# andgoldschmidt/MPC4quantum

Hardware: AMD Instinct MI355X
Metric: MPC horizon-steps/sec across batch (3-level transmon, T=40) (higher is better)
Workload: dtype f64

## Files before the change

### mpc4quantum_amd/csrc/build.py

```python
import argparse
import os
import re
import subprocess
import sys
from concurrent.futures import ThreadPoolExecutor

HERE = os.path.dirname(os.path.abspath(__file__))
PKG = os.path.dirname(HERE)
OBJ = os.path.join(HERE, "build")
LIB = os.path.join(PKG, "libm4q_hip.so")
LIB_GEN = os.path.join(PKG, "libm4q_hip_gen.so")
HIPCC = os.environ.get("HIPCC", "/opt/rocm/bin/hipcc")
COMMON = ["--offload-arch=gfx950", "-O3", "-std=c++17", "-fPIC", "-fvisibility=hidden", "-Wno-unused-command-line-argument"]
HEADERS = ["m4q_device.h", "m4q_dpp_gen.h", "m4q_mpc.h", "m4q_tile.h", "m4q_tile3.h", "m4q_tile_opnd.h", "m4q_rollout_pair.h", "m4q_args.h", "m4q_paths.h", "m4q_lift.h", "m4q_noise.h", "m4q_fit.h", "m4q_fit_qr.h", "m4q_online.h", "m4q_grad.h", "m4q_plant_lin.h", "m4q_plant_qp.h", "m4q_plant_step.h", "m4q_rollout_multi.h", "m4q_robust_host.h", "m4q_feedback.h", "m4q_observe.h", "m4q_shapes.inc",
           os.path.join("..", "..", "include", "m4q.h")]
STAMP = os.path.join(OBJ, "flags.stamp")


def shapes():
    txt = open(os.path.join(HERE, "m4q_shapes.inc")).read()
    return [(int(a), int(b), int(c), "plant-only" in rest)
            for a, b, c, rest in re.findall(r"^M4Q_SHAPE\((\d+),\s*(\d+),\s*(\d+)\)(.*)$", txt, re.M)]


def stale(target, sources):
    if not os.path.exists(target):
        return True
    t = os.path.getmtime(target)
    return any(os.path.getmtime(s) > t for s in sources)


def run(cmd):
    res = subprocess.run(cmd, stdout=subprocess.PIPE, stderr=subprocess.STDOUT, text=True)
    if res.returncode != 0:
        sys.stderr.write(" ".join(cmd) + "\n" + res.stdout)
        raise RuntimeError("hipcc failed")
    return res.stdout


def build(force=False, jobs=None, extra=()):
    os.makedirs(OBJ, exist_ok=True)
    hdrs = [os.path.join(HERE, h) for h in HEADERS]
    gen = os.path.join(HERE, "m4q_dpp_gen.h")
    if stale(gen, [os.path.join(HERE, "gen_dpp.py")]):
        text = run([sys.executable, os.path.join(HERE, "gen_dpp.py")])
        if not os.path.exists(gen) or open(gen).read() != text:
            with open(gen, "w") as f:
                f.write(text)
    want = " ".join(extra)
    have = open(STAMP).read() if os.path.exists(STAMP) else None
    if have != want:
        force = True
    jobs_list = []
    objs = []
    gen_objs = []
    for nx, nu, order, plant_only in shapes():
        obj = os.path.join(OBJ, "kernels_%d_%d_%d.o" % (nx, nu, order))
        objs.append(obj)
        src = os.path.join(HERE, "m4q_kernels.hip")
        dims = ["-DM4Q_NX=%d" % nx, "-DM4Q_NU=%d" % nu, "-DM4Q_ORDER=%d" % order]
        if force or stale(obj, [src] + hdrs):
            jobs_list.append([HIPCC] + COMMON + list(extra) + dims + (["-DM4Q_PLANT_ONLY"] if plant_only else []) + ["-c", src, "-o", obj])
        d = {4: 2, 9: 3, 16: 4}.get(nx)
        if d and not plant_only:
            gobj = os.path.join(OBJ, "kernelsg_%d_%d_%d.o" % (nx, nu, order))
            gen_objs.append(gobj)
            if force or stale(gobj, [src] + hdrs):
# ... 35 lines not shown
```

### mpc4quantum_amd/csrc/m4q_capi.hip

```cpp
#include <hip/hip_runtime.h>
#include <dlfcn.h>
#include <rccl/rccl.h>

#include <algorithm>
#include <cfloat>
#include <cmath>
#include <complex>
#include <cstdlib>
#include <cstdarg>
#include <cstdio>
#include <cstring>
#include <deque>
#include <mutex>
#include <string>
#include <vector>

#include "../../include/m4q.h"
#include "m4q_args.h"
#include "m4q_lift.h"
#include "m4q_robust_host.h"

namespace m4q {
struct cplx { double re, im; };
}
// ... 824 lines not shown
  s->noise_seed = seed;
  s->noise_member_base = member_base;
  s->noise_mode = mode;
  return 0;
}

int m4q_session_sync(m4q_session* s) {
  if (!s) return fail(M4Q_E_BADARG, "m4q_session_sync: null session");
  HIP_TRY(hipStreamSynchronize(s->stream));
  return check_watchdog(s);
}

int m4q_session_set_codes(m4q_session* s, const int32_t* codes) {
  if (!s || !codes) return fail(M4Q_E_BADARG, "m4q_session_set_codes: bad argument");
  HIP_TRY(hipMemcpyAsync(s->f[M4Q_F_CODES].p, codes, (size_t)s->B * 4, hipMemcpyHostToDevice, s->stream));
  HIP_TRY(hipStreamSynchronize(s->stream));
  return check_watchdog(s);
}

int m4q_session_kernel_ms(m4q_session* s, double* total_ms, int32_t* launches) {
  if (!s) return fail(M4Q_E_BADARG, "m4q_session_kernel_ms: null session");
  HIP_TRY(hipStreamSynchronize(s->stream));
  double tot = s->folded_ms;
  int n = s->folded_n;
  s->folded_ms = 0.0;
  s->folded_n = 0;
  for (auto& pr : s->pending) {
    float ms = 0.f;
    HIP_TRY(hipEventElapsedTime(&ms, pr.first, pr.second));
    tot += ms;
    ++n;
    (void)hipEventDestroy(pr.first);
    (void)hipEventDestroy(pr.second);
  }
  s->pending.clear();
  if (total_ms) *total_ms = tot;
  if (launches) *launches = n;
  return check_watchdog(s);
}

int m4q_session_qp_stats(m4q_session* s, int64_t* out6) {
  if (!s || !out6) return fail(M4Q_E_BADARG, "m4q_session_qp_stats: bad argument");
  HIP_TRY(hipStreamSynchronize(s->stream));
  unsigned long long q[24];
  HIP_TRY(hipMemcpy(q, s->queue.p, sizeof(q), hipMemcpyDeviceToHost));
  for (int i = 0; i < 6; ++i) out6[i] = (int64_t)q[1 + i];
  if (std::getenv("M4Q_QP_TRACE"))
    fprintf(stderr, "m4q: exact QP: %llu row sweeps in %llu wavefront passes (x4 rows = %llu): lane efficiency %.2f\n", q[2], q[7],
            4 * q[7], q[7] ? (double)q[2] / (4.0 * (double)q[7]) : 0.0);
  if (std::getenv("M4Q_PHASE_TRACE")) {
    static const char* names[16] = {"draw/resume", "backward | exact: adjoint pass", "forward", "handover", "line search", "step done (plant)", "publish",
                                    "passes", "guess update", "passes with a line search",
                                    "step: bookkeeping, us | exact: pinned sweep", "step: plant to xs | exact: policy rollout",
                                    "exact: ratio rollout", "step: exit, rest | exact: blend", "exact: open rollout",
                                    "exact: bookkeeping + copies"};
    unsigned long long tot = 0;
    for (int i = 0; i < 16; ++i) tot += (i == 7 || i == 9) ? 0 : q[8 + i];
    for (int i = 0; i < 16; ++i)
      fprintf(stderr, "m4q phase %-44s %14llu %s  %5.1f %%\n", names[i], q[8 + i], (i == 7 || i == 9) ? "     " : "ticks",
              (i != 7 && i != 9 && tot) ? 100.0 * (double)q[8 + i] / (double)tot : 0.0);
  }
  return check_watchdog(s);
}

int m4q_session_info(const m4q_session* s, int64_t* hbm_bytes, int32_t* grid, int32_t* lds_bytes) {
  if (!s) return fail(M4Q_E_BADARG, "m4q_session_info: null session");
  int64_t tot = 0;
  for (int i = 0; i < M4Q_F_COUNT; ++i) tot += (int64_t)s->f[i].bytes;
  tot += (int64_t)(s->wsXg.bytes + s->wsUg.bytes + s->wsG.bytes);
  if (hbm_bytes) *hbm_bytes = tot;
  const m4q::Path path = s->path();
  if (grid) *grid = path == m4q::PATH_SG ? s->grid_sg : s->grid;
  if (lds_bytes) *lds_bytes = s->mpc_ops->mpc_lds_bytes(s->prob.plant_kind, path, (s->prob.qp_flags & M4Q_QP_EXACT_BOX) != 0);
  return 0;
}

int m4q_linearize_batch(int32_t B, int32_t dim_x, int32_t dim_u, int32_t order, int32_t T, const double* models,
                        int32_t model_per_instance, const double* X, const double* U, double* A_ls, double* B_ls,
                        double* Delta_ls) {
  const m4q::ShapeOps* sh = find_shape(dim_x, dim_u, order);
  if (!sh) return fail(M4Q_E_UNSUPPORTED, "no kernel for dim_x=%d dim_u=%d order=%d", dim_x, dim_u, order);
  if (B <= 0 || T <= 0 || !models || !X || !U || !A_ls || !B_ls || !Delta_ls) return fail(M4Q_E_BADARG, "m4q_linearize_batch: bad argument");
  if (int rc = need_device()) return rc;
  const size_t n = dim_x, m = dim_u, P = sh->np, BT = (size_t)B * T;
  const Extent mdl(B, model_per_instance, n * n * (1 + P));
  Stage st;
  m4q::LinArgs a{};
  a.B = B; a.T = T;
  a.models = st.in<cplx>(models, mdl.count); a.model_stride = mdl.stride;
  a.X = st.in<cplx>(X, BT * n); a.U = st.in<double>(U, BT * m);
  a.A_ls = st.out<cplx>(A_ls, BT * n * n); a.B_ls = st.out<cplx>(B_ls, BT * n * m); a.D_ls = st.out<cplx>(Delta_ls, BT * n);
  if (st.error()) return st.error();
  return st.finish(sh->launch_linearize(a, nullptr), "linearize");
}

int m4q_quad_program_batch(int32_t B, int32_t dim_x, int32_t dim_u, int32_t T, int32_t qp_flags, double sat, double du,
                           const double* x_init, const double* X_bm, const double* U_bm, int32_t bm_per_instance,
                           const double* Q_ls, const double* R_ls, const double* A_ls, const double* B_ls,
                           const double* Delta_ls, const double* u_prev, double* X_opt, double* U_opt, double* cost,
                           double* gains) {
  const m4q::ShapeOps* sh = find_shape_any_order(dim_x, dim_u);
  if (!sh) return fail(M4Q_E_UNSUPPORTED, "no kernel for dim_x=%d dim_u=%d", dim_x, dim_u);
  if (B <= 0 || T <= 0 || !x_init || !X_bm || !U_bm || !Q_ls || !R_ls || !A_ls || !B_ls || !X_opt || !U_opt || !cost)
    return fail(M4Q_E_BADARG, "m4q_quad_program_batch: bad argument");
  if (!(sat > 0)) return fail(M4Q_E_BADARG, "sat must be positive");
  if (int rc = check_qp_flags(qp_flags)) return rc;
  if (int rc = need_device()) return rc;
  const size_t n = dim_x, m = dim_u, BT = (size_t)B * T, BT1 = (size_t)B * (T + 1);
  const Extent xbm(B, bm_per_instance, (size_t)(T + 1) * n), ubm(B, bm_per_instance, (size_t)T * m);
  Stage st;
  m4q::QpArgs a{};
  a.B = B; a.T = T; a.flags = qp_flags; a.sat = sat; a.du = du;
  a.x_init = st.in<cplx>(x_init, (size_t)B * n);
// ... 1188 lines not shown
```

### mpc4quantum_amd/csrc/m4q_kernels.hip

```cpp
#define M4Q_KERNEL_TU 1
#include "m4q_args.h"
#include "m4q_mpc.h"
#include "m4q_feedback.h"
#include "m4q_fit.h"
#include "m4q_fit_qr.h"
#include "m4q_online.h"
#include "m4q_grad.h"
#include "m4q_plant_lin.h"
#include "m4q_plant_qp.h"
#include "m4q_noise.h"
#include "m4q_observe.h"
#include "m4q_tile3.h"

#ifndef M4Q_NX
#error "compile with -DM4Q_NX -DM4Q_NU -DM4Q_ORDER"
#endif
#if defined(M4Q_PLANT_ONLY) || defined(M4Q_VARIANT_GEN)
#define M4Q_NO_AUX 1
#endif

#define M4Q_CAT_(a, b, c, d) a##b##_##c##_##d
#define M4Q_CAT(a, b, c, d) M4Q_CAT_(a, b, c, d)

namespace m4q {
namespace M4Q_CAT(shape_, M4Q_NX, M4Q_NU, M4Q_ORDER) {

constexpr int NX = M4Q_NX;
constexpr int NU = M4Q_NU;
constexpr int ORDER = M4Q_ORDER;
constexpr int DD = (NX == 4) ? 2 : (NX == 9) ? 3 : (NX == 16) ? 4 : 1;
constexpr bool SQUARE = DD * DD == NX;
constexpr int DQ = fourth_root(NX);
constexpr bool QUARTIC = DQ > 0;
constexpr int NP = PowTab<NU, ORDER>::NP;
constexpr int PITCH = ModelPitch<NX>::value;
constexpr int MODEL_ELEMS = (1 + NP) * NX * PITCH;
constexpr int SCRATCH_ELEMS = (SQUARE ? DD * DD : 0) + 2 * NX;
constexpr int ROWS = 4;
constexpr bool HAS_TILE = SQUARE && ORDER == 1 && NX - 1 <= 8;
constexpr bool HAS_SG = SQUARE && ORDER == 1 && NX == 16;

constexpr int WAVES = NX <= 9 ? 2 : 1;
#define M4Q_OCC __attribute__((amdgpu_waves_per_eu(WAVES, 8)))

extern __shared__ __align__(16) unsigned char m4q_lds_raw[];

template <int N, class S>
__device__ __forceinline__ void stage_model(S* dst, const M4Q_GLOBAL S* src, int jj) {
  constexpr int W = N * (1 + NP);
#pragma unroll 1
  for (int e = jj; e < N * W; e += 16) {
    const int i = e / W;
    const int pk = e - i * W;
    const int p = pk / N;
    const int k = pk - p * N;
    dst[ModelPitch<N>::at(p, i, k)] = gld(src, e);
  }
}

struct LaneGeo {
  int g, jj, j;
  bool lane_ok;
  __device__ __forceinline__ LaneGeo() {
    const int lane = threadIdx.x;
    g = lane >> 4;
// ... 76 lines not shown

template <int NS>
struct ExactTile {
  static constexpr bool enabled = true;
  const double* lds_models;
  volatile M4Q_LDS double* tgb; volatile M4Q_LDS int* tiw; volatile M4Q_LDS double* tpin;
  GView Xg, Ug, gains;
  const double* Q; const double* Qf; const double* R;
  unsigned sX, sU, sG;
  int g, jj;
  __device__ __forceinline__ void sweep(int T, const Window& win, const PinCtx<NU>& pin, bool going) const {
    if (jj == 0) {
      tiw[g * TILE_IO_WORDS + 0] = going ? 1 : 0;
      tiw[g * TILE_IO_WORDS + 1] = (int)win.xbm.off;
      tiw[g * TILE_IO_WORDS + 2] = (int)win.ubm.off;
      tiw[g * TILE_IO_WORDS + 3] = (int)pin.stat.off;
#pragma unroll
      for (int k = 0; k < NU; ++k) { tpin[g * TILE_PIN_DOUBLES + k] = pin.lo0[k]; tpin[g * TILE_PIN_DOUBLES + 3 + k] = pin.hi0[k]; }
    }
    wave_sync();
    TileBackwardB<NS, NU, ORDER, true> ts;
    const int mb = ts.L.mb;
    const int dm = mb - g;
    ts.mdl = lds_models + mb * model_elems<NS>();
    ts.T = T;
    ts.Xg = Xg; ts.Xg.off = Xg.off + (unsigned)(dm * (int)(sX * sizeof(double)));
    ts.Ug = Ug; ts.Ug.off = Ug.off + (unsigned)(dm * (int)(sU * sizeof(double)));
    ts.gains = gains; ts.gains.off = gains.off + (unsigned)(dm * (int)(sG * sizeof(double)));
    ts.xbm = win.xbm; ts.xbm.off = (unsigned)tiw[mb * TILE_IO_WORDS + 1];
    ts.ubm = win.ubm; ts.ubm.off = (unsigned)tiw[mb * TILE_IO_WORDS + 2];
    ts.stat = pin.stat; ts.stat.off = (unsigned)tiw[mb * TILE_IO_WORDS + 3];
    ts.sat = pin.box.sat;
    ts.Q = Q; ts.Qf = Qf; ts.R = R;
    ts.gb = tgb + mb * TILE_GB_DOUBLES;
    const bool run_t = tiw[mb * TILE_IO_WORDS + 0] != 0;
    ts.backward(run_t);
    wave_sync();
  }
};

constexpr int TC_MIN_N = 8;
constexpr int XCUTS[] = {4, 7, 12};
constexpr int NXC = (int)(sizeof(XCUTS) / sizeof(int));
constexpr int WAVES_SG = 2;
constexpr int WAVES_TILE = 2;
template <class S, int PLANT, bool EXACT, bool TL, bool TILE, bool SG>
constexpr PrioMap prio_map() {
  if (TILE && !EXACT && NX == 9 && PLANT == PLANT_HAMILTONIAN) return PrioMap{0, 1, 1, 1, 1, 1};
  return PrioMap{0, 0, 0, 0, 0, 0};
}
template <bool EXACT>
constexpr bool shift_in_update() {
  return !EXACT;
}
#if defined(M4Q_DEV_PHASE_CLOCK)
#define M4Q_PHASE_FLUSH() if (threadIdx.x == 0) { for (int i = 0; i < 16; ++i) __hip_atomic_fetch_add((M4Q_GLOBAL unsigned long long*)kargs()->queue + 8 + i, pc.acc[i], __ATOMIC_RELAXED, __HIP_MEMORY_SCOPE_AGENT); }
#else
#define M4Q_PHASE_FLUSH()
#endif
#define M4Q_PHASE_DECL PhaseClock pc;
#define M4Q_PHASE_MARK(i) pc.mark(i);
#define M4Q_PHASE_MARK_CLIP(i) if constexpr (!EXACT) pc.mark(i);
template <class S, int PLANT, bool EXACT, bool TL = false, bool TILE = false, bool SG = false>
__global__ __launch_bounds__(64) __attribute__((amdgpu_waves_per_eu(SG ? WAVES_SG : TILE ? WAVES_TILE : WAVES, 8))) void mpc_kernel(MpcArgs) {
  static_assert(!TL || (sizeof(S) == sizeof(double) && SQUARE), "the traceless path is a real path of a d x d density matrix");
  static_assert(!TILE || (TL && !EXACT && ORDER == 1), "tile sweep: clipped solve on the traceless real coordinates, order-1 libraries");
  static_assert(!SG || (TL && !TILE && !EXACT && ORDER == 1), "shared generators: the clipped traceless kernel of an order-1 library");
  constexpr int NS = TL ? NX - 1 : NX;
  using Prov = FusedProv<S, NS, NU, ORDER, SG>;
  cplx* scratch = reinterpret_cast<cplx*>(m4q_lds_raw);
  S* lds = reinterpret_cast<S*>(scratch + ROWS * SCRATCH_ELEMS);
  const LaneGeo L;
  const int g = L.g, jj = L.jj;
  const int j = jj < NS ? jj : NS - 1;
  const int jio = L.j;
  const bool lane_ok = jj < NS, lane_io = L.lane_ok;
  double tau = 0.0;
  constexpr bool QTR = cost_transposed<S, NS, EXACT>();
  constexpr int MODEL_K = SG ? NS * ModelPitch<NS>::value : model_elems<NS>(), COST_K = cost_elems<NS>() + (QTR ? 2 * NS * NS : 0);
  S* mdl = lds + g * MODEL_K;
  S* mdn = lds + ROWS * MODEL_K;
  scratch += g * SCRATCH_ELEMS;
  S* ldsQ = lds + model_lds_elems<NS, SG>();
  double* ldsW = reinterpret_cast<double*>(ldsQ + COST_K);
  volatile M4Q_LDS unsigned long long* wd_slot = (volatile M4Q_LDS unsigned long long*)(ldsW + WLS_DOUBLES);
  RowStash<S> stash;
  stash.w = (volatile M4Q_LDS int*)(ldsW + WLS_DOUBLES + 1);
  stash.xm = stash_x_in_scratch<S, SG>() ? (volatile M4Q_LDS double*)m4q_lds_raw : (volatile M4Q_LDS double*)(stash.w + ROWS * STASH_INTS);
  volatile M4Q_LDS double* tgb = stash.xm + 64 * 2;
  volatile M4Q_LDS int* tiw = (volatile M4Q_LDS int*)(tgb + ROWS * TILE_GB_DOUBLES);
  volatile M4Q_LDS double* tpin = (volatile M4Q_LDS double*)(tiw + ROWS * TILE_IO_WORDS);
  volatile M4Q_LDS double* timg = (volatile M4Q_LDS double*)(tiw + ROWS * TILE_IO_WORDS);
  int T0, flags;
  bool ls_diag, two_phase;
  int n_pieces;
  auto piece_cut = [](int i) __attribute__((always_inline)) {
    int v = 2;
#pragma unroll
    for (int k = 0; k < NXC; ++k)
      if (i == k + 2) v = XCUTS[k];
    return v;
  };
  auto piece_of = [&](int begin, int step_begin) __attribute__((always_inline)) {
    int ph = begin == step_begin ? 0 : 1;
#pragma unroll
    for (int k = 0; k < NXC; ++k)
      if (begin == XCUTS[k] && begin != step_begin) ph = k + 2;
    return ph;
  };
  {
    KArgs* a = kargs();
    T0 = a->T;
    flags = a->flags;
    const M4Q_GLOBAL S* gQ = (const M4Q_GLOBAL S*)a->Q;
    const M4Q_GLOBAL S* gQf = (const M4Q_GLOBAL S*)a->Qf;
    const M4Q_GLOBAL S* gR = (const M4Q_GLOBAL S*)a->R;
    for (int e = threadIdx.x; e < 2 * NS * NS + NU * NU; e += 64)
      ldsQ[e] = e < NS * NS ? gld(gQ, e) : (e < 2 * NS * NS ? gld(gQf, e - NS * NS) : gld(gR, e - 2 * NS * NS));
    if constexpr (QTR) {
      for (int e = threadIdx.x; e < 2 * NS * NS; e += 64) {
        const int blk = e / (NS * NS), r = (e / NS) % NS, c = e % NS;
        ldsQ[cost_elems<NS>() + e] = gld(blk ? gQf : gQ, c * NS + r);
      }
    }
    if constexpr (SG) {
      for (int e = threadIdx.x; e < NP * NS * NS; e += 64) {
        const int p = e / (NS * NS), r = (e / NS) % NS, c = e % NS;
        mdn[ModelPitch<NS>::at(p, r, c)] = gld((const M4Q_GLOBAL S*)a->gens, NS * NS + e);
      }
    }
    ls_diag = a->Wls != nullptr;
    if (ls_diag) {
      for (int e = threadIdx.x; e < WLS_DOUBLES; e += 64) ldsW[e] = gld(a->Wls, e);
    }
    two_phase = a->step_begin < 2 && a->step_end > 2;
    n_pieces = two_phase ? 2 : 1;
    if constexpr (EXACT) {
#pragma unroll
      for (int i = 0; i < NXC; ++i)
        if (two_phase && a->step_end > XCUTS[i]) ++n_pieces;
    }
    if (threadIdx.x == 0) *wd_slot = __builtin_amdgcn_s_memrealtime() + a->deadline_ticks;
  }
  CostRef<S, QTR> cost;
  cost.Q = ldsQ; cost.Qf = ldsQ + NS * NS; cost.q_stride = 0; cost.R = ldsQ + 2 * NS * NS; cost.r_stride = 0;
  if constexpr (QTR) { cost.QT = ldsQ + cost_elems<NS>(); cost.QfT = cost.QT + NS * NS; }
  const unsigned sX = (unsigned)(T0 + 1) * NS, sU = (unsigned)T0 * NU, sG = (unsigned)T0 * (NS + 1) * NU;
  const unsigned sXc = (unsigned)(T0 + 1) * NX;
  constexpr bool PIECE_RAW = sizeof(S) == sizeof(double);
  constexpr bool MASK_IDLE = NS < 16 && !EXACT && !TILE;
  constexpr PrioMap PRIO = prio_map<S, PLANT, EXACT, TL, TILE, SG>();
  constexpr bool PRIO_ON = PRIO.any();
  constexpr bool SHIFT_IN_UPDATE = shift_in_update<EXACT>();
  static_assert(!EXACT || !PRIO_ON, "the exact solve's phases are those of box_qp_iterate: no levels there yet");
  GView Xg, Ug, Xo, Uo, gains, Xalt, Ualt, pin_stat;
  {
    KArgs* a = kargs();
    const long wsb = blockIdx.x;
    M4Q_GLOBAL S* wX = (M4Q_GLOBAL S*)a->ws_Xg;
    Xg = gview(wX, wsb * ROWS * sX, g * sX);
    Ug = gview(a->ws_Ug, wsb * ROWS * sU, g * sU);
    Xo = gview(wX, wsb * ROWS * sX, g * sX + gridDim.x * ROWS * sX);
    Uo = gview(a->ws_Ug, wsb * ROWS * sU, g * sU + gridDim.x * ROWS * sU);
    gains = gview((M4Q_GLOBAL S*)a->ws_gains, wsb * ROWS * sG, g * sG);
    Xalt = gview(wX, wsb * ROWS * sX, g * sX + 2 * gridDim.x * ROWS * sX);
    Ualt = gview(a->ws_Ug, wsb * ROWS * sU, g * sU + 2 * gridDim.x * ROWS * sU);
    pin_stat = gview(a->ws_Ug, wsb * ROWS * sU, g * sU + 3 * gridDim.x * ROWS * sU);
  }
  const bool band = (flags & QP_DU_BAND) != 0;

  long b = 0;
  bool active = false, need_new = true, pending = false;
  int step = 0, iter = 0, code = 0, done_steps = 0;
  int row_begin = 0, row_end = 0;
  S x_cur = zero_of<S>();
  S x_meas = zero_of<S>();
  double uprev[NU];
#pragma unroll
  for (int k = 0; k < NU; ++k) uprev[k] = 0.0;
  double gsc[SG ? NU : 1];
#pragma unroll
  for (int k = 0; k < (SG ? NU : 1); ++k) gsc[k] = 1.0;
  BoxQpRow qp;
  int qp_passes = 0;
  unsigned xt_off = 0, ut_off = 0, op0_off = 0, ops_off = 0;
  wave_sync();
  M4Q_PHASE_DECL

  while (true) {
    int T = T0;
    asm volatile("" : "+s"(T));
    asm volatile("" : "+v"(Xg.off), "+v"(Ug.off), "+v"(Xo.off), "+v"(Uo.off), "+v"(gains.off));
    if constexpr (EXACT) asm volatile("" : "+v"(Xalt.off), "+v"(Ualt.off), "+v"(pin_stat.off));
    Prov prov;
    prov.mdl = mdl; prov.Xg = Xg; prov.Ug = Ug; prov.j = j;
    if constexpr (SG) prov.mdn = mdn;

    if (__builtin_amdgcn_s_memrealtime() > *wd_slot) {
      if (threadIdx.x == 0) __hip_atomic_store(kargs()->queue + 1, 1, __ATOMIC_RELAXED, __HIP_MEMORY_SCOPE_AGENT);
      break;
    }
    M4Q_PHASE_MARK(3)
    if (__any(need_new || pending)) {
      KArgs* a = kargs();
      const int B = a->B, n_items = n_pieces * B;
      const int step_begin = a->step_begin, step_end = a->step_end, mf = a->measure_freq;
      const long sXs = (long)(a->n_steps + 1) * NX, sUs = (long)a->n_steps * NU;
      int nb = 0;
      if (need_new && jj == 0) nb = __hip_atomic_fetch_add(a->queue, 1, __ATOMIC_RELAXED, __HIP_MEMORY_SCOPE_AGENT);
      nb = row_bcast_int(nb);
      if (need_new) {
        need_new = false;
        if (nb < n_items) {
          const int ph = nb / B;
          b = nb - ph * B;
          row_begin = ph == 0 ? step_begin : piece_cut(ph);
          row_end = ph == n_pieces - 1 ? step_end : piece_cut(ph + 1);
          pending = true;
        }
      }
      int ready = 1;
      const bool later = two_phase && row_begin != step_begin;
      if (pending && later && jj == 0)
        ready = __hip_atomic_load(a->head_done + b, __ATOMIC_RELAXED, __HIP_MEMORY_SCOPE_AGENT) >= piece_of(row_begin, step_begin) ? 1 : 0;
      ready = row_bcast_int(ready);
      const bool fresh = pending && ready != 0;
      if (__any(fresh && later)) {
        __builtin_amdgcn_fence(__ATOMIC_ACQUIRE, "agent");
        asm volatile("s_waitcnt vmcnt(0)" ::: "memory");
      }
      if (fresh) { pending = false; active = true; }
      wave_sync();
      if (fresh) {
        if constexpr (SG) {
          const M4Q_GLOBAL double* sc = a->scales + b * (1 + NU);
          const double s0 = gld(sc, 0);
#pragma unroll
          for (int k = 0; k < NU; ++k) gsc[k] = gld(sc, 1 + k);

#pragma unroll 1
          for (int e = jj; e < NS * NS; e += 16) {
            const int r = e / NS, c = e - r * NS;
            mdl[ModelPitch<NS>::at(0, r, c)] = fma(s0, gld((const M4Q_GLOBAL S*)a->gens, e), r == c ? 1.0 : 0.0);
          }
        } else {
          stage_model<NS>(mdl, (const M4Q_GLOBAL S*)a->models + b * a->model_stride, jj);
        }
        xt_off = (unsigned)(b * a->xt_stride) * (unsigned)sizeof(S);
        ut_off = (unsigned)(b * a->ut_stride) * (unsigned)sizeof(double);
        op0_off = (unsigned)(b * a->op0_stride) * (unsigned)sizeof(cplx);
        ops_off = (unsigned)(b * a->ops_stride) * (unsigned)sizeof(cplx);
        step = row_begin;
        iter = 0;
        code = 0;
        done_steps = 0;
        if (row_begin <= 1) {
          GView u0 = gview(a->u_targ, 0, 0);
          u0.off = ut_off;
#pragma unroll
          for (int k = 0; k < NU; ++k) uprev[k] = u0.ld<double>(k);
        }
      }
      if (__any(fresh && row_begin == 0)) {
        if (fresh && row_begin == 0) {
          const S x0 = gld((const M4Q_GLOBAL S*)a->x0s, b * NS + j);
          x_cur = x0;
          x_meas = x0;
          if (lane_ok) {
#pragma unroll 8
            for (int t = 0; t <= T; ++t) Xg.st<S>(t * NS + j, x0);
          }
          if (lane_io) gst(a->xs, b * sXs + jio, gld(a->x0c, b * NX + jio));
          for (int e = jj; e < T * NU; e += 16) Ug.st<double>(e, 0.0);
        }
        if constexpr (TL) {
          double t0 = 0.0;
          const cplx xc = (fresh && row_begin == 0) ? gld(a->x0c, b * NX + jio) : czero();
          (void)Basis<S, TL>::template to_state<NX, DD>(xc, scratch, j, jj, t0);
          if (fresh && row_begin == 0) tau = t0;
        }
      }
      if (__any(fresh && row_begin != 0)) {
        const bool rs = fresh && row_begin != 0;
        const bool rs_raw = PIECE_RAW && rs && later;
        double tdum = 0.0, tnew = 0.0;
        if (__any(rs && !rs_raw)) {
          for (int t0 = 0; t0 <= T; t0 += 8) {
            cplx v[8];
#pragma unroll
            for (int q = 0; q < 8; ++q) v[q] = (rs && !rs_raw) ? gld(a->Xg, b * sXc + (t0 + q <= T ? t0 + q : T) * NX + jio) : czero();
            __builtin_amdgcn_sched_barrier(0);
#pragma unroll
            for (int q = 0; q < 8; ++q) {
              if (t0 + q <= T) {
                const S r = Basis<S, TL>::template to_state<NX, DD>(v[q], scratch, j, jj, tdum);
                if (rs && !rs_raw && lane_ok) Xg.st<S>((t0 + q) * NS + j, r);
              }
            }
          }
        }
        if constexpr (PIECE_RAW) {
          if (rs_raw) {
            const M4Q_GLOBAL double* raw = (const M4Q_GLOBAL double*)(a->Xg + b * sXc);
            const int count = (T + 1) * NS;
            if constexpr (NS % 2 == 0) {
              constexpr int U = 6;
              for (int e0 = 2 * jj; e0 < count; e0 += 32 * U) {
                d2_t v[U];
#pragma unroll
                for (int u = 0; u < U; ++u) v[u] = *reinterpret_cast<const M4Q_GLOBAL d2_t*>(raw + (e0 + 32 * u < count ? e0 + 32 * u : count - 2));
                __builtin_amdgcn_sched_barrier(0);
#pragma unroll
                for (int u = 0; u < U; ++u) {
                  if (e0 + 32 * u < count) {
                    const double r[2] = {v[u].x, v[u].y};
                    stn<2>(Xg, e0 + 32 * u, r);
                  }
                }
              }
            } else {
              constexpr int U = 12;
              for (int e0 = jj; e0 < count; e0 += 16 * U) {
                double v[U];
#pragma unroll
                for (int u = 0; u < U; ++u) v[u] = gld(raw, e0 + 16 * u < count ? e0 + 16 * u : count - 1);
                __builtin_amdgcn_sched_barrier(0);
#pragma unroll
                for (int u = 0; u < U; ++u)
                  if (e0 + 16 * u < count) Xg.st<double>(e0 + 16 * u, v[u]);
              }
            }
          }
        }
        const cplx xc = rs ? gld(a->xs, b * sXs + (long)row_begin * NX + jio) : czero();
        const S r = Basis<S, TL>::template to_state<NX, DD>(xc, scratch, j, jj, tdum);
        const cplx xm = rs ? gld(a->xs, b * sXs + (long)(row_begin / mf) * mf * NX + jio) : czero();
        const S rm = Basis<S, TL>::template to_state<NX, DD>(xm, scratch, j, jj, tnew);
        if (rs) {
          x_cur = r;
          x_meas = rm;
          tau = tnew;
          for (int e = jj; e < T * NU; e += 16) Ug.st<double>(e, gld(a->Ug, b * sU + e));
          code = gld(a->codes, b);
          done_steps = gld(a->steps_done, b);
#pragma unroll
          for (int k = 0; k < NU; ++k) uprev[k] = row_begin > 1 ? gld(a->us, b * sUs + (long)(row_begin - 1) * NU + k) : uprev[k];
          if (code != 0) step = row_end;
        }
      }
      wave_sync();
    }
    M4Q_PHASE_MARK(0)
    if (!__any(active || pending)) {
      M4Q_PHASE_FLUSH()
      if (EXACT && threadIdx.x == 0)
        __hip_atomic_fetch_add((M4Q_GLOBAL unsigned long long*)kargs()->queue + 7, (unsigned long long)qp_passes, __ATOMIC_RELAXED,
                               __HIP_MEMORY_SCOPE_AGENT);
      break;
    }
    if (!__any(active)) {
      __builtin_amdgcn_s_sleep(8);
      continue;
    }
    issue_prio<PRIO_ON && PRIO.sweep != 0, PRIO.sweep>();
    const bool running = active && step < row_end;
    if constexpr (SG) {
#pragma unroll
      for (int k = 0; k < NU; ++k) prov.sc[k] = gsc[k];
    }

    stash.put_int(g, jj, 0, (int)(b & 0xffffffff));
    stash.put_int(g, jj, 1, (int)(b >> 32));
    stash.put_int(g, jj, 2, code);
    stash.put_int(g, jj, 3, done_steps);
    stash.put_int(g, jj, 4, row_begin);
    stash.put_int(g, jj, 5, (active ? 1 : 0) | (need_new ? 2 : 0) | (pending ? 4 : 0));
    stash.put_int(g, jj, 6, (int)op0_off);
    stash.put_int(g, jj, 7, (int)ops_off);
    stash.put_x(x_meas);
    double uapp[NU];
#pragma unroll
    for (int k = 0; k < NU; ++k) uapp[k] = 0.0;
    double chk = 0.0;
    bool solved = running;
    bool capped = false;
    bool use_ls;
    Window win;
    {
      KArgs* a = kargs();
      const int w = step <= 1 ? 0 : step - 1;
      win.xbm = gview((const M4Q_GLOBAL S*)a->x_targ, 0, 0);
      win.xbm.off = xt_off + (unsigned)w * NS * (unsigned)sizeof(S);
      win.ubm = gview(a->u_targ, 0, 0);
      win.ubm.off = ut_off + (unsigned)w * NU * (unsigned)sizeof(double);
      const double sat = a->sat, du = a->du;
      double lo0[NU], hi0[NU];
#pragma unroll
      for (int k = 0; k < NU; ++k) {
        const double up = uprev[k];
        lo0[k] = band ? up - du : -sat;
// ... 394 lines not shown
        }
        if (shift_late && jj < NU) {
          for (int t0 = 0; t0 + 1 < T; t0 += 8) {
            double buf[8];
#pragma unroll
            for (int q = 0; q < 8; ++q) buf[q] = Ug.ld<double>((t0 + q + 1 < T ? t0 + q + 1 : T - 1) * NU + jj);
#pragma unroll
            for (int q = 0; q < 8; ++q)
              if (t0 + q + 1 < T) Ug.st<double>((t0 + q) * NU + jj, buf[q]);
          }
        }
      }
      if (ok) done_steps = step + 1;
      if (step_done) {
        iter = 0;
        step = fail ? row_end : step + 1;
      }
      if constexpr (PLANT != PLANT_NONE) {
        const int xmode = a->exit_mode;
        if (xmode != 0) {
          const int s0 = step - 1;
          const bool prev = (xmode & EXIT_PREV) != 0;
          const cplx x = !ok ? czero() : (prev && s0 == 0) ? gld(a->x0c, b * NX + jio)
                                                           : gld(a->xs, b * sXs + (long)(prev ? s0 : s0 + 1) * NX + jio);
          const cplx d = csub(x, ok ? gld(a->exit_target, b * a->exit_tstride + jio) : czero());
          const M4Q_GLOBAL cplx* Wr = a->exit_W + jio * NX;
          cplx y = czero();
          static_for<0, NX>([&](auto k) { cmac(y, gld(Wr, decltype(k)::value), bcast<decltype(k)::value>(d)); });
          const double q = rowsum<NX>(dot_re(d, y));
          const double thr = ok ? gld(a->exit_thr, b * a->exit_thr_stride) : 0.0;
          if (ok && ((xmode & EXIT_ABOVE) ? q > thr : q < thr)) {
            code = 1;
            done_steps = s0;
            step = row_end;
          }
        }
      }
      wave_sync();
      if constexpr (PLANT == PLANT_NONE) {
        const bool carry = ok && step < row_end;
        const cplx xc = carry ? gld(a->xs, b * sXs + (long)step * NX + jio) : czero();
        double tnew = 0.0;
        const S rn = Basis<S, TL>::template to_state<NX, DD>(xc, scratch, j, jj, tnew);
        if (carry) { x_cur = rn; if constexpr (TL) tau = tnew; }
      }
      M4Q_PHASE_MARK_CLIP(13)
    }

    issue_prio<PRIO_ON && PRIO.publish != PRIO.step_done, PRIO.publish>();
    M4Q_PHASE_MARK(5)
    const bool finished = active && step >= row_end;
    if (__any(finished)) {
      KArgs* a = kargs();
      const bool last_piece = row_end == a->step_end;
      if constexpr (TL && NS % 2 == 0) {
        if (finished && last_piece) {
          for (int t = jj; t <= T; t += 16) {
            double r[NS];
#pragma unroll
            for (int h = 0; h < NS / 2; ++h) {
              double p2[2];
              ldn<2>(Xg, (unsigned)(t * NS + 2 * h), p2);
              r[2 * h] = p2[0]; r[2 * h + 1] = p2[1];
            }
            cplx out[NX];
            tl_node_to_complex<NX, DD>(r, tau, out);
#pragma unroll
            for (int c = 0; c < NX; ++c) gst(a->Xg, b * sXc + t * NX + c, out[c]);
          }
        }
      } else if (__any(finished && (!PIECE_RAW || last_piece))) {
        for (int t0 = 0; t0 <= T; t0 += 8) {
          S v[8];
#pragma unroll
          for (int q = 0; q < 8; ++q) v[q] = Xg.ld<S>((t0 + q <= T ? t0 + q : T) * NS + j);
          __builtin_amdgcn_sched_barrier(0);
#pragma unroll
          for (int q = 0; q < 8; ++q) {
            if (t0 + q <= T) {
              const cplx xc = Basis<S, TL>::template to_complex<NX, DD>(v[q], tau, scratch, j, jj);
              if (finished && (!PIECE_RAW || last_piece) && lane_io) gst(a->Xg, b * sXc + (t0 + q) * NX + jio, xc);
            }
          }
        }
      }
      if constexpr (PIECE_RAW) {
        if (finished && !last_piece) {
          M4Q_GLOBAL double* raw = (M4Q_GLOBAL double*)(a->Xg + b * sXc);
          const int count = (T + 1) * NS;
          if constexpr (NS % 2 == 0) {
            constexpr int U = 6;
            for (int e0 = 2 * jj; e0 < count; e0 += 32 * U) {
              double v[U][2];
#pragma unroll
              for (int u = 0; u < U; ++u) ldn<2>(Xg, e0 + 32 * u < count ? e0 + 32 * u : count - 2, v[u]);
              __builtin_amdgcn_sched_barrier(0);
#pragma unroll
              for (int u = 0; u < U; ++u) {
                if (e0 + 32 * u < count) {
                  d2_t w; w.x = v[u][0]; w.y = v[u][1];
                  *reinterpret_cast<M4Q_GLOBAL d2_t*>(raw + e0 + 32 * u) = w;
                }
              }
            }
          } else {
            constexpr int U = 12;
            for (int e0 = jj; e0 < count; e0 += 16 * U) {
              double v[U];
#pragma unroll
              for (int u = 0; u < U; ++u) v[u] = Xg.ld<double>(e0 + 16 * u < count ? e0 + 16 * u : count - 1);
              __builtin_amdgcn_sched_barrier(0);
#pragma unroll
              for (int u = 0; u < U; ++u)
                if (e0 + 16 * u < count) gst(raw, e0 + 16 * u, v[u]);
            }
          }
        }
      }
      if (finished) {
        for (int e = jj; e < T * NU; e += 16) gst(a->Ug, b * sU + e, Ug.ld<double>(e));
        if (jj == 0) {
          gst(a->codes, b, code);
          gst(a->steps_done, b, done_steps);
        }
      }
      if (two_phase && __any(finished && row_end != kargs()->step_end)) {
        asm volatile("s_waitcnt vmcnt(0)" ::: "memory");
        wave_sync();
        __builtin_amdgcn_fence(__ATOMIC_RELEASE, "agent");
        asm volatile("s_waitcnt vmcnt(0)" ::: "memory");
        if (finished && row_end != a->step_end && jj == 0)
          __hip_atomic_store(a->head_done + b, piece_of(row_begin, a->step_begin) + 1, __ATOMIC_RELAXED, __HIP_MEMORY_SCOPE_AGENT);
      }
      if (finished) {
        active = false;
        need_new = true;
      }
      wave_sync();
    }
    M4Q_PHASE_MARK(6)
    pc.count(7);
    issue_prio<PRIO_ON, 0>();
  }
}

#ifndef M4Q_VARIANT_GEN
struct RollOut {
  int N, xs_mode, q_mode;
  M4Q_GLOBAL cplx* xs; M4Q_GLOBAL double* q;
  const M4Q_GLOBAL cplx* Wr;
  cplx f;
  long b;
  int j;
  bool st, st0;
  __device__ __forceinline__ RollOut(const RollArgs& a, long b_, int j_, bool st_, bool st0_)
      : N(a.N), xs_mode(a.xs_mode), q_mode(a.q_mode), xs(a.xs), q(a.q), Wr(a.W + j_ * NX), f(czero()), b(b_), j(j_), st(st_), st0(st0_) {
    if (q_mode != 0) f = gld(a.target, b * a.target_stride + j);
  }
  __device__ __forceinline__ void put(int t, cplx x) const {
    const bool last = t == N;
    if (xs_mode == 2) {
      if (st) gst(xs, (b * (N + 1) + t) * NX + j, x);
    } else if (xs_mode == 1 && last) {
      if (st) gst(xs, b * NX + j, x);
    }
    if (q_mode == 2 || (q_mode == 1 && last)) {
      const double qv = quad_figure<NX>(csub(x, f), Wr);
      if (st0) gst(q, q_mode == 2 ? b * (N + 1) + t : b, qv);
    }
  }
};
struct RollCtl {
  const M4Q_GLOBAL double* u;
// ... 1328 lines not shown
```

Baseline: 4.766 billion.

## Batch item handover loads and stores into issued-together trips

```diff
diff --git a/mpc4quantum_amd/csrc/build.py b/mpc4quantum_amd/csrc/build.py
--- a/mpc4quantum_amd/csrc/build.py
+++ b/mpc4quantum_amd/csrc/build.py
@@ -12,7 +12,7 @@
 LIB_GEN = os.path.join(PKG, "libm4q_hip_gen.so")
 HIPCC = os.environ.get("HIPCC", "/opt/rocm/bin/hipcc")
 COMMON = ["--offload-arch=gfx950", "-O3", "-std=c++17", "-fPIC", "-fvisibility=hidden", "-Wno-unused-command-line-argument"]
-HEADERS = ["m4q_device.h", "m4q_dpp_gen.h", "m4q_mpc.h", "m4q_tile.h", "m4q_tile3.h", "m4q_tile_opnd.h", "m4q_rollout_pair.h", "m4q_args.h", "m4q_paths.h", "m4q_lift.h", "m4q_noise.h", "m4q_fit.h", "m4q_fit_qr.h", "m4q_online.h", "m4q_grad.h", "m4q_plant_lin.h", "m4q_plant_qp.h", "m4q_plant_step.h", "m4q_rollout_multi.h", "m4q_robust_host.h", "m4q_feedback.h", "m4q_observe.h", "m4q_shapes.inc",
+HEADERS = ["m4q_device.h", "m4q_dpp_gen.h", "m4q_mpc.h", "m4q_tile.h", "m4q_tile3.h", "m4q_tile_opnd.h", "m4q_handover.h", "m4q_rollout_pair.h", "m4q_args.h", "m4q_paths.h", "m4q_lift.h", "m4q_noise.h", "m4q_fit.h", "m4q_fit_qr.h", "m4q_online.h", "m4q_grad.h", "m4q_plant_lin.h", "m4q_plant_qp.h", "m4q_plant_step.h", "m4q_rollout_multi.h", "m4q_robust_host.h", "m4q_feedback.h", "m4q_observe.h", "m4q_shapes.inc",
            os.path.join("..", "..", "include", "m4q.h")]
 STAMP = os.path.join(OBJ, "flags.stamp")
 
diff --git a/mpc4quantum_amd/csrc/m4q_capi.hip b/mpc4quantum_amd/csrc/m4q_capi.hip
--- a/mpc4quantum_amd/csrc/m4q_capi.hip
+++ b/mpc4quantum_amd/csrc/m4q_capi.hip
@@ -900,13 +900,20 @@
     static const char* names[16] = {"draw/resume", "backward | exact: adjoint pass", "forward", "handover", "line search", "step done (plant)", "publish",
                                     "passes", "guess update", "passes with a line search",
                                     "step: bookkeeping, us | exact: pinned sweep", "step: plant to xs | exact: policy rollout",
-                                    "exact: ratio rollout", "step: exit, rest | exact: blend", "exact: open rollout",
-                                    "exact: bookkeeping + copies"};
+                                    "passes with an item drawn | exact: ratio rollout", "step: exit, rest | exact: blend",
+                                    "passes with an item published | exact: open rollout",
+                                    "draw: ticket, flag, acquire | exact: bookkeeping + copies"};
+    const bool exact = q[7] != 0;
+    auto is_count = [&](int i) { return i == 7 || i == 9 || (!exact && (i == 12 || i == 14)); };
     unsigned long long tot = 0;
-    for (int i = 0; i < 16; ++i) tot += (i == 7 || i == 9) ? 0 : q[8 + i];
-    for (int i = 0; i < 16; ++i)
-      fprintf(stderr, "m4q phase %-44s %14llu %s  %5.1f %%\n", names[i], q[8 + i], (i == 7 || i == 9) ? "     " : "ticks",
-              (i != 7 && i != 9 && tot) ? 100.0 * (double)q[8 + i] / (double)tot : 0.0);
+    for (int i = 0; i < 16; ++i) tot += is_count(i) ? 0 : q[8 + i];
+    for (int i = 0; i < 16; ++i) {
+      std::string name = names[i];
+      const size_t bar = name.find(" | ");
+      if (bar != std::string::npos) name = exact ? name.substr(bar + 3) : name.substr(0, bar);
+      fprintf(stderr, "m4q phase %-44s %14llu %s  %5.1f %%\n", name.c_str(), q[8 + i], is_count(i) ? "     " : "ticks",
+              (!is_count(i) && tot) ? 100.0 * (double)q[8 + i] / (double)tot : 0.0);
+    }
   }
   return check_watchdog(s);
 }
diff --git a/mpc4quantum_amd/csrc/m4q_handover.h b/mpc4quantum_amd/csrc/m4q_handover.h
--- /dev/null
+++ b/mpc4quantum_amd/csrc/m4q_handover.h
@@ -0,0 +1,94 @@
+#pragma once
+#include "m4q_device.h"
+#include "m4q_mpc.h"
+
+namespace m4q {
+
+constexpr int HANDOVER_MODEL_VGPRS = 8;
+constexpr int HANDOVER_XG_PAIRS = 6;
+constexpr int HANDOVER_XG_SINGLES = 12;
+constexpr int HANDOVER_UG_PAIRS = 3;
+constexpr int HANDOVER_UG_SINGLES = 6;
+constexpr int HANDOVER_NODE_ROUNDS = 3;
+
+template <bool PAIR, int U>
+struct FlatTrip {
+  static constexpr int STEP = PAIR ? 2 : 1, SPAN = 16 * STEP * U;
+  double v[U][STEP];
+  static __device__ __forceinline__ int elem(int e0, int u, int jj) { return e0 + 16 * STEP * u + STEP * jj; }
+  __device__ __forceinline__ void load(const GView& src, int e0, int jj, int count) {
+#pragma unroll
+    for (int u = 0; u < U; ++u) {
+      const int e = elem(e0, u, jj);
+      ldn<STEP>(src, (unsigned)(e < count ? e : count - STEP), v[u]);
+    }
+  }
+  __device__ __forceinline__ void load(const M4Q_GLOBAL double* src, int e0, int jj, int count) {
+#pragma unroll
+    for (int u = 0; u < U; ++u) {
+      const int e = elem(e0, u, jj);
+      const M4Q_GLOBAL double* p = src + (e < count ? e : count - STEP);
+      if constexpr (PAIR) {
+        const d2_t w = *reinterpret_cast<const M4Q_GLOBAL d2_t*>(p);
+        v[u][0] = w.x; v[u][1] = w.y;
+      } else {
+        v[u][0] = *p;
+      }
+    }
+  }
+  __device__ __forceinline__ void store(const GView& dst, int e0, int jj, int count, bool ok) const {
+#pragma unroll
+    for (int u = 0; u < U; ++u) {
+      const int e = elem(e0, u, jj);
+      if (ok && e < count) stn<STEP>(dst, (unsigned)e, v[u]);
+    }
+  }
+  __device__ __forceinline__ void store(M4Q_GLOBAL double* dst, int e0, int jj, int count, bool ok) const {
+#pragma unroll
+    for (int u = 0; u < U; ++u) {
+      const int e = elem(e0, u, jj);
+      if (ok && e < count) {
+        if constexpr (PAIR) {
+          d2_t w; w.x = v[u][0]; w.y = v[u][1];
+          *reinterpret_cast<M4Q_GLOBAL d2_t*>(dst + e) = w;
+        } else {
+          dst[e] = v[u][0];
+        }
+      }
+    }
+  }
+};
+template <int NU> using UgTrip = FlatTrip<NU % 2 == 0, NU % 2 == 0 ? HANDOVER_UG_PAIRS : HANDOVER_UG_SINGLES>;
+
+template <class S, int N, int P>
+struct ModelTrip {
+  static constexpr int W = N * (1 + P), COUNT = N * W;
+  static constexpr int PER = HANDOVER_MODEL_VGPRS / (int)(sizeof(S) / 4);
+  static constexpr int TRIPS = (COUNT + 16 * PER - 1) / (16 * PER);
+  static constexpr int SLOTS_LAST = (COUNT - 16 * PER * (TRIPS - 1) + 15) / 16;
+  S v[PER];
+  __device__ __forceinline__ void load(const M4Q_GLOBAL S* src, int jj, int trip) {
+#pragma unroll
+    for (int u = 0; u < PER; ++u) {
+      if (trip + 1 < TRIPS || u < SLOTS_LAST) {
+        const int e = 16 * (PER * trip + u) + jj;
+        v[u] = gld(src, e < COUNT ? e : COUNT - 1);
+      }
+    }
+  }
+  __device__ __forceinline__ void store(S* dst, int jj, int trip, bool ok) const {
+#pragma unroll
+    for (int u = 0; u < PER; ++u) {
+      if (trip + 1 < TRIPS || u < SLOTS_LAST) {
+        const int e = 16 * (PER * trip + u) + jj;
+        const int i = e / W;
+        const int pk = e - i * W;
+        const int p = pk / N;
+        const int k = pk - p * N;
+        if (ok && e < COUNT) dst[ModelPitch<N>::at(p, i, k)] = v[u];
+      }
+    }
+  }
+};
+
+}
diff --git a/mpc4quantum_amd/csrc/m4q_kernels.hip b/mpc4quantum_amd/csrc/m4q_kernels.hip
--- a/mpc4quantum_amd/csrc/m4q_kernels.hip
+++ b/mpc4quantum_amd/csrc/m4q_kernels.hip
@@ -11,6 +11,7 @@
 #include "m4q_noise.h"
 #include "m4q_observe.h"
 #include "m4q_tile3.h"
+#include "m4q_handover.h"
 
 #ifndef M4Q_NX
 #error "compile with -DM4Q_NX -DM4Q_NU -DM4Q_ORDER"
@@ -193,6 +194,10 @@
 template <bool EXACT>
 constexpr bool shift_in_update() {
   return !EXACT;
+}
+template <int PLANT, bool TILE>
+constexpr bool batch_handover() {
+  return TILE && PLANT != PLANT_GENERATOR;
 }
 #if defined(M4Q_DEV_PHASE_CLOCK)
 #define M4Q_PHASE_FLUSH() if (threadIdx.x == 0) { for (int i = 0; i < 16; ++i) __hip_atomic_fetch_add((M4Q_GLOBAL unsigned long long*)kargs()->queue + 8 + i, pc.acc[i], __ATOMIC_RELAXED, __HIP_MEMORY_SCOPE_AGENT); }
@@ -293,6 +298,8 @@
   constexpr PrioMap PRIO = prio_map<S, PLANT, EXACT, TL, TILE, SG>();
   constexpr bool PRIO_ON = PRIO.any();
   constexpr bool SHIFT_IN_UPDATE = shift_in_update<EXACT>();
+  constexpr bool BATCH = batch_handover<PLANT, TILE>();
+  static_assert(!BATCH || (!SG && PIECE_RAW), "the batched item change: per-member models, the raw guess between items");
   static_assert(!EXACT || !PRIO_ON, "the exact solve's phases are those of box_qp_iterate: no levels there yet");
   GView Xg, Ug, Xo, Uo, gains, Xalt, Ualt, pin_stat;
   {
@@ -372,6 +379,31 @@
       }
       if (fresh) { pending = false; active = true; }
       wave_sync();
+      M4Q_PHASE_MARK_CLIP(15)
+      if constexpr (!EXACT) { if (__any(fresh)) pc.count(12); }
+      ModelTrip<S, NS, NP> hin_model;
+      S hin_x0 = zero_of<S>();
+      cplx hin_xa = czero();
+      double hin_u[NU];
+#pragma unroll
+      for (int k = 0; k < NU; ++k) hin_u[k] = 0.0;
+      int jl = jj;
+      constexpr bool U_LATE = ModelTrip<S, NS, NP>::TRIPS > 1;
+#define M4Q_HIN_PU (row_begin > 1 ? (const M4Q_GLOBAL double*)a->us + (b * sUs + (long)(row_begin - 1) * NU) : a->u_targ + b * a->ut_stride)
+      if constexpr (BATCH) {
+        asm volatile("" : "+v"(jl));
+        if (__any(fresh)) {
+          hin_model.load((const M4Q_GLOBAL S*)a->models + b * a->model_stride, jl, 0);
+          hin_x0 = gld((const M4Q_GLOBAL S*)a->x0s, b * NS + j);
+          const M4Q_GLOBAL cplx* pa = row_begin == 0 ? a->x0c + b * NX : (const M4Q_GLOBAL cplx*)a->xs + (b * sXs + (long)row_begin * NX);
+          hin_xa = gld(pa, jio);
+          if constexpr (!U_LATE) {
+#pragma unroll
+            for (int k = 0; k < NU; ++k) hin_u[k] = gld(M4Q_HIN_PU, k);
+          }
+        }
+        __builtin_amdgcn_sched_barrier(0);
+      }
       if (fresh) {
         if constexpr (SG) {
           const M4Q_GLOBAL double* sc = a->scales + b * (1 + NU);
@@ -384,6 +416,22 @@
             const int r = e / NS, c = e - r * NS;
             mdl[ModelPitch<NS>::at(0, r, c)] = fma(s0, gld((const M4Q_GLOBAL S*)a->gens, e), r == c ? 1.0 : 0.0);
           }
+        } else if constexpr (BATCH) {
+          const M4Q_GLOBAL S* src = (const M4Q_GLOBAL S*)a->models + b * a->model_stride;
+#pragma unroll
+          for (int trip = 0; trip < ModelTrip<S, NS, NP>::TRIPS; ++trip) {
+            if (trip > 0) {
+              hin_model.load(src, jl, trip);
+              if (U_LATE && trip == 1) {
+#pragma unroll
+                for (int k = 0; k < NU; ++k) hin_u[k] = gld(M4Q_HIN_PU, k);
+              }
+              __builtin_amdgcn_sched_barrier(0);
+            }
+            hin_model.store(mdl, jl, trip, true);
+          }
+#pragma unroll
+          for (int k = 0; k < NU; ++k) uprev[k] = hin_u[k];
         } else {
           stage_model<NS>(mdl, (const M4Q_GLOBAL S*)a->models + b * a->model_stride, jj);
         }
@@ -395,7 +443,8 @@
         iter = 0;
         code = 0;
         done_steps = 0;
-        if (row_begin <= 1) {
+#undef M4Q_HIN_PU
+        if (!BATCH && row_begin <= 1) {
           GView u0 = gview(a->u_targ, 0, 0);
           u0.off = ut_off;
 #pragma unroll
@@ -404,19 +453,19 @@
       }
       if (__any(fresh && row_begin == 0)) {
         if (fresh && row_begin == 0) {
-          const S x0 = gld((const M4Q_GLOBAL S*)a->x0s, b * NS + j);
+          const S x0 = BATCH ? hin_x0 : gld((const M4Q_GLOBAL S*)a->x0s, b * NS + j);
           x_cur = x0;
           x_meas = x0;
           if (lane_ok) {
 #pragma unroll 8
             for (int t = 0; t <= T; ++t) Xg.st<S>(t * NS + j, x0);
           }
-          if (lane_io) gst(a->xs, b * sXs + jio, gld(a->x0c, b * NX + jio));
+          if (lane_io) gst(a->xs, b * sXs + jio, BATCH ? hin_xa : gld(a->x0c, b * NX + jio));
           for (int e = jj; e < T * NU; e += 16) Ug.st<double>(e, 0.0);
         }
         if constexpr (TL) {
           double t0 = 0.0;
-          const cplx xc = (fresh && row_begin == 0) ? gld(a->x0c, b * NX + jio) : czero();
+          const cplx xc = (fresh && row_begin == 0) ? (BATCH ? hin_xa : gld(a->x0c, b * NX + jio)) : czero();
           (void)Basis<S, TL>::template to_state<NX, DD>(xc, scratch, j, jj, t0);
           if (fresh && row_begin == 0) tau = t0;
         }
@@ -445,7 +494,7 @@
             const M4Q_GLOBAL double* raw = (const M4Q_GLOBAL double*)(a->Xg + b * sXc);
             const int count = (T + 1) * NS;
             if constexpr (NS % 2 == 0) {
-              constexpr int U = 6;
+              constexpr int U = HANDOVER_XG_PAIRS;
               for (int e0 = 2 * jj; e0 < count; e0 += 32 * U) {
                 d2_t v[U];
 #pragma unroll
@@ -460,7 +509,7 @@
                 }
               }
             } else {
-              constexpr int U = 12;
+              constexpr int U = HANDOVER_XG_SINGLES;
               for (int e0 = jj; e0 < count; e0 += 16 * U) {
                 double v[U];
 #pragma unroll
@@ -473,20 +522,44 @@
             }
           }
         }
-        const cplx xc = rs ? gld(a->xs, b * sXs + (long)row_begin * NX + jio) : czero();
+        const cplx xc = rs ? (BATCH ? hin_xa : gld(a->xs, b * sXs + (long)row_begin * NX + jio)) : czero();
         const S r = Basis<S, TL>::template to_state<NX, DD>(xc, scratch, j, jj, tdum);
-        const cplx xm = rs ? gld(a->xs, b * sXs + (long)(row_begin / mf) * mf * NX + jio) : czero();
+        cplx hin_xm = czero();
+        int hin_code = 0, hin_done = 0;
+        UgTrip<NU> hin_ug;
+        if constexpr (BATCH) {
+          hin_xm = gld(a->xs, b * sXs + (long)(row_begin / mf) * mf * NX + jio);
+          hin_code = gld(a->codes, b);
+          hin_done = gld(a->steps_done, b);
+          hin_ug.load(a->Ug + b * sU, 0, jl, T * NU);
+          __builtin_amdgcn_sched_barrier(0);
+        }
+        const cplx xm = rs ? (BATCH ? hin_xm : gld(a->xs, b * sXs + (long)(row_begin / mf) * mf * NX + jio)) : czero();
         const S rm = Basis<S, TL>::template to_state<NX, DD>(xm, scratch, j, jj, tnew);
         if (rs) {
           x_cur = r;
           x_meas = rm;
           tau = tnew;
-          for (int e = jj; e < T * NU; e += 16) Ug.st<double>(e, gld(a->Ug, b * sU + e));
-          code = gld(a->codes, b);
-          done_steps = gld(a->steps_done, b);
-#pragma unroll
-          for (int k = 0; k < NU; ++k) uprev[k] = row_begin > 1 ? gld(a->us, b * sUs + (long)(row_begin - 1) * NU + k) : uprev[k];
+          if constexpr (!BATCH) {
+            for (int e = jj; e < T * NU; e += 16) Ug.st<double>(e, gld(a->Ug, b * sU + e));
+          }
+          code = BATCH ? hin_code : gld(a->codes, b);
+          done_steps = BATCH ? hin_done : gld(a->steps_done, b);
+          if constexpr (!BATCH) {
+#pragma unroll
+            for (int k = 0; k < NU; ++k) uprev[k] = row_begin > 1 ? gld(a->us, b * sUs + (long)(row_begin - 1) * NU + k) : uprev[k];
+          }
           if (code != 0) step = row_end;
+        }
+        if constexpr (BATCH) {
+          const int cu = T * NU;
+          for (int e0 = 0; e0 < cu; e0 += UgTrip<NU>::SPAN) {
+            if (e0 > 0) {
+              hin_ug.load(a->Ug + b * sU, e0, jl, cu);
+              __builtin_amdgcn_sched_barrier(0);
+            }
+            hin_ug.store(Ug, e0, jl, cu, rs);
+          }
         }
       }
       wave_sync();
@@ -987,8 +1060,44 @@
     const bool finished = active && step >= row_end;
     if (__any(finished)) {
       KArgs* a = kargs();
+      if constexpr (!EXACT) pc.count(14);
       const bool last_piece = row_end == a->step_end;
-      if constexpr (TL && NS % 2 == 0) {
+      UgTrip<NU> pub_ug;
+      int jl = jj;
+      if constexpr (BATCH) {
+        asm volatile("" : "+v"(jl));
+        pub_ug.load(Ug, 0, jl, T * NU);
+        __builtin_amdgcn_sched_barrier(0);
+      }
+      if constexpr (BATCH && TL && NS % 2 == 0) {
+        if (finished && last_piece) {
+          constexpr int R = HANDOVER_NODE_ROUNDS;
+          for (int tb = 0; tb <= T; tb += 16 * R) {
+            double r[R][NS];
+#pragma unroll
+            for (int q = 0; q < R; ++q) {
+              const int t = tb + 16 * q + jl <= T ? tb + 16 * q + jl : T;
+#pragma unroll
+              for (int h = 0; h < NS / 2; ++h) {
+                double p2[2];
+                ldn<2>(Xg, (unsigned)(t * NS + 2 * h), p2);
+                r[q][2 * h] = p2[0]; r[q][2 * h + 1] = p2[1];
+              }
+            }
+            __builtin_amdgcn_sched_barrier(0);
+#pragma unroll
+            for (int q = 0; q < R; ++q) {
+              const int t = tb + 16 * q + jl;
+              if (t <= T) {
+                cplx out[NX];
+                tl_node_to_complex<NX, DD>(r[q], tau, out);
+#pragma unroll
+                for (int c = 0; c < NX; ++c) gst(a->Xg, b * sXc + t * NX + c, out[c]);
+              }
+            }
+          }
+        }
+      } else if constexpr (TL && NS % 2 == 0) {
         if (finished && last_piece) {
           for (int t = jj; t <= T; t += 16) {
             double r[NS];
@@ -1024,7 +1133,7 @@
           M4Q_GLOBAL double* raw = (M4Q_GLOBAL double*)(a->Xg + b * sXc);
           const int count = (T + 1) * NS;
           if constexpr (NS % 2 == 0) {
-            constexpr int U = 6;
+            constexpr int U = HANDOVER_XG_PAIRS;
             for (int e0 = 2 * jj; e0 < count; e0 += 32 * U) {
               double v[U][2];
 #pragma unroll
@@ -1039,7 +1148,7 @@
               }
             }
           } else {
-            constexpr int U = 12;
+            constexpr int U = HANDOVER_XG_SINGLES;
             for (int e0 = jj; e0 < count; e0 += 16 * U) {
               double v[U];
 #pragma unroll
@@ -1052,8 +1161,20 @@
           }
         }
       }
+      if constexpr (BATCH) {
+        const int cu = T * NU;
+        for (int e0 = 0; e0 < cu; e0 += UgTrip<NU>::SPAN) {
+          if (e0 > 0) {
+            pub_ug.load(Ug, e0, jl, cu);
+            __builtin_amdgcn_sched_barrier(0);
+          }
+          pub_ug.store(a->Ug + b * sU, e0, jl, cu, finished);
+        }
+      }
       if (finished) {
-        for (int e = jj; e < T * NU; e += 16) gst(a->Ug, b * sU + e, Ug.ld<double>(e));
+        if constexpr (!BATCH) {
+          for (int e = jj; e < T * NU; e += 16) gst(a->Ug, b * sU + e, Ug.ld<double>(e));
+        }
         if (jj == 0) {
           gst(a->codes, b, code);
           gst(a->steps_done, b, done_steps);
```

Result: no change. 4.771 billion (median of 4 runs) (+0.1%).
